# tavildar/Polar

Measured on AMD Instinct MI355X. Metric: codewords/s (N=2048 K=1024 L=32 LLR-SCL), higher is better.
Workload: dtype f64

## Files before the change

### include/polar_amd_debug.h

```cpp
#ifndef POLAR_AMD_DEBUG_H
#define POLAR_AMD_DEBUG_H
#include "polar_amd.h"
#ifdef __cplusplus
extern "C" {
#endif

int polar_debug_set(polar_code_t *h, const char *key, long value);
long polar_debug_get(const polar_code_t *h, const char *key);
int polar_debug_comm_inits(void);
int polar_debug_weak_leaves(const polar_code_t *h);
void *polar_debug_scratch_ptr(polar_code_t *h);

#ifdef __cplusplus
}
#endif
#endif
```

### polar_amd/csrc/polar_debug.cpp

```cpp
#include "polar_multi.h"
#include "polar_amd_debug.h"

extern "C" {

int polar_debug_weak_leaves(const polar_code_t *h) { return polar_get_weak_leaves(h); }

int polar_debug_set(polar_code_t *h, const char *key, long value) {
    if (!h || !key) return fail(POLAR_E_ARG, "NULL argument");
    polar_code::Knobs &k = h->knobs;
    const std::string s(key);
    if (s == "mode_override") { if (value < -1 || value > 2) return fail(POLAR_E_ARG, "mode_override must be -1 (none), 0, 1 or 2"); k.mode_override = (int)value; }
    else if (s == "sc_no_fold") k.sc_no_fold = value != 0;
    else if (s == "no_tables") k.no_tables = value != 0;
    else if (s == "no_fuse_front") k.no_fuse_front = value != 0;
    else if (s == "no_prefix") h->prefix_on = (value == 0);
    else if (s == "no_rccl") { k.no_rccl = value != 0; multi_release(h, false); }
    else if (s == "force_rccl") { k.force_rccl = value != 0; multi_release(h, false); }
#ifdef POLAR_TEST_HOOKS
    else if (s == "host_fail_alloc") k.host_fail_alloc = value;
    else if (s == "share_device") { k.share_device = value != 0; multi_release(h, false); }
    else if (s == "fail_device") k.fail_device = (int)value;
    else if (s == "fail_collective") k.fail_collective = (int)value;
#endif
    else if (s == "lat_max_b") k.lat_max_b = value;
    else if (s == "host_pipe_min_bytes") k.host_pipe_min_bytes = value;
    else if (s == "host_chunk_bytes") k.host_chunk_bytes = value;
    else if (s == "host_lanes") { if (value < 0 || value > HostPipe::kMaxLanes) return fail(POLAR_E_ARG, "host_lanes must be 0 (default) or 1 .. %d", HostPipe::kMaxLanes); k.host_lanes = value; }
    else if (s == "host_ramp") k.host_ramp = value;
    else if (s == "host_prefault") { if (value < -1 || value > 16) return fail(POLAR_E_ARG, "host_prefault must be -1 (none), 0 (default) or 1 .. 16 threads"); k.host_prefault = value; }
    else if (s == "host_threads") { if (value < 0) return fail(POLAR_E_ARG, "host_threads must be >= 0"); k.host_threads = value; }
    else if (s == "multi_grace_s") { if (value < 0) return fail(POLAR_E_ARG, "multi_grace_s must be >= 0"); k.multi_grace_s = value; }
#ifdef POLAR_TEST_HOOKS
    else if (s == "force_workers") { k.force_workers = value != 0; multi_release(h, false); }
    else if (s == "stall_device") k.stall_device = (int)value;
    else if (s == "stall_ms") { if (value < 0) return fail(POLAR_E_ARG, "stall_ms must be >= 0"); k.stall_ms = value; }
#endif
    else if (s == "multi_timeout_s") { if (value < 0) return fail(POLAR_E_ARG, "multi_timeout_s must be >= 0 (0 = no watchdog)"); k.multi_timeout_s = value; }
    else return fail(POLAR_E_ARG, "polar_debug_set: unknown key '%s'", key);
    drop_clones(h);
    return POLAR_OK;
}
void *polar_debug_scratch_ptr(polar_code_t *h) { return h ? (void *)h->d_llr_scr.p : nullptr; }
long polar_debug_get(const polar_code_t *h, const char *key) {
    if (!key) return -1;
    const std::string s(key);
    if (s == "allocs") return (long)g_allocs.load();
    if (s == "comm_inits") return (long)polar_debug_comm_inits();
// ... 4 lines not shown
#else
        return 0;
#endif
    }
    if (s == "weak_leaves") return h->weak_leaves;
    if (s == "mode_override") return h->knobs.mode_override;
    if (s == "last_rounds") return h->last_rounds;
    if (s == "last_round_max_per_device") return h->last_round_max_per_device;
    if (s == "worker_threads_started") return h->worker_threads_started;
    if (s.compare(0, 9, "round_us_") == 0) {
        if (h->round_us.empty()) return 0;
        std::vector<long> v(h->round_us);
        if (s == "round_us_count") return (long)v.size();
        if (s == "round_us_first") return v.front();
        std::sort(v.begin(), v.end());
        if (s == "round_us_min") return v.front();
        if (s == "round_us_max") return v.back();
        if (s == "round_us_median") return v[v.size() / 2];
        return -1;
    }
    if (s == "multi_poisoned") return h->multi_poisoned ? 1 : 0;
    if (s == "host_chunks") return h->hpipe ? h->hpipe->last_chunks : 0;
    if (s == "host_chunk_cw") return h->hpipe ? h->hpipe->last_chunk_cw : 0;
    if (s == "host_lanes") return h->hpipe ? h->hpipe->last_lanes : 0;
    if (s == "host_threads") return h->hpipe ? h->hpipe->last_threads : 0;
    if (s == "host_us_copy_in") return h->hpipe ? h->hpipe->us_copy_in : 0;
    if (s == "host_us_wait") return h->hpipe ? h->hpipe->us_wait : 0;
    if (s == "host_us_copy_out") return h->hpipe ? h->hpipe->us_copy_out : 0;
    if (s == "host_us_total") return h->hpipe ? h->hpipe->us_total : 0;
    return -1;
}
int polar_debug_comm_inits(void) { return g_comm_inits.load(); }

}
```

### polar_amd/csrc/polar_decode.cpp

```cpp
#include "polar_host.h"

namespace {

size_t scratch_budget(const polar_code *h) {
    size_t budget = (size_t)24 << 30, free_b = 0, total_b = 0;
    if (hipMemGetInfo(&free_b, &total_b) == hipSuccess) budget = std::min(budget, (free_b + h->d_llr_scr.cap * sizeof(double)) / 2);
    return std::max(budget, (size_t)64 << 20);
}
template <typename Ensure>
int grid_that_fits(const polar_code *h, long want, size_t per_wave, Ensure ensure, int *grid_out) {
    long grid = want;
    if ((size_t)want * per_wave > h->d_llr_scr.cap * sizeof(double)) grid = std::max<long>(1, std::min<long>(want, (long)(scratch_budget(h) / per_wave)));
    for (;;) {
        const int rc = ensure((int)grid);
        if (rc != POLAR_E_NOMEM || grid <= 64) { *grid_out = (int)grid; return rc; }
        (void)hipGetLastError();
        grid /= 2;
    }
}

}

extern "C" {

int polar_decode_scl_llr_batch_dev(polar_code_t *h, const double *d_llr, long B, int L, uint8_t *d_out,
                                   double *d_pm, void *stream) {
    return polar_decode_scl_llr_batch_dev_ev(h, d_llr, B, L, d_out, d_pm, stream, nullptr, nullptr);
}

}

bool polar_host::use_sc_lat(const polar_code *h, long B) {
    return h->n <= polar_sc_lat_max_log() && polar_sc_lat_lds_bytes(h->N, (int)h->sc_lat_ops.size()) <= h->lds_per_block &&
           h->knobs.lat_max_b >= 0 && B <= (h->knobs.lat_max_b ? h->knobs.lat_max_b : 2048);
}

extern "C" {

int polar_decode_scl_llr_batch_dev_ev(polar_code_t *h, const double *d_llr, long B, int L, uint8_t *d_out,
                                      double *d_pm, void *stream, void *ev_start, void *ev_stop) {
    return decode_impl(h, d_llr, 0, B, nullptr, L, d_out, d_pm, stream, ev_start, ev_stop);
}

}

int polar_host::decode_impl(polar_code *h, const void *d_llr, int llr_f32, long B, const unsigned int *n_dev, int L, uint8_t *d_out,
                            double *d_pm, void *stream, void *ev_start, void *ev_stop, int phase, int *deferred) {
    if (!h || !d_llr || !d_out) return fail(POLAR_E_ARG, "NULL argument");
    if (deferred) *deferred = 0;
    if (L < 1 || L > POLAR_MAX_LIST) return fail(POLAR_E_ARG, "list size %d out of range [1, %d]", L, POLAR_MAX_LIST);
    if (B < 0) return fail(POLAR_E_ARG, "negative batch");
    if (B == 0) return POLAR_OK;
    DevGuard dg_;
    int rc = ensure_device(h, dg_);
    if (rc) return rc;
    const int gs = pow2ceil(L);
    const int G = 64 / gs;
    int wpc = h->waves_per_cu ? h->waves_per_cu : 16;
    int lds_log_auto = 0;
    if (!h->waves_per_cu && !h->lds_log && gs >= 16 && (B + G - 1) / G <= (long)h->num_cu * 4 &&
        polar_decode_lds_bytes(5, 1) <= h->lds_per_block) { wpc = 4; lds_log_auto = 5; }
    const int pipe = (wpc > 8) ? 0 : 1;
    int lds_log = h->lds_log ? h->lds_log : (lds_log_auto ? lds_log_auto : (pipe ? 4 : 3));
    const int wpb = polar_decode_waves_per_block(pipe);
    const size_t lds = polar_decode_lds_bytes(lds_log, pipe);
    const int max_blocks_by_lds = (int)(h->lds_per_block / lds);
    if (max_blocks_by_lds < 1) return fail(POLAR_E_ARG, "lds_log %d does not fit the LDS", lds_log);
    if (wpc > max_blocks_by_lds * wpb) wpc = max_blocks_by_lds * wpb;
    long groups = (B + G - 1) / G;
    long maxgrid = (long)h->num_cu * wpc;
    int grid = (int)std::min(groups, maxgrid);
    grid = ((grid + wpb - 1) / wpb) * wpb;
    const int SL = 1 << lds_log;
    const size_t big = (h->N > 2 * SL) ? (size_t)(h->N - 2 * SL) : 0;
    const size_t cwords = (h->N >= 128) ? (size_t)(h->N / 32 - 2) : 0;
    if ((size_t)grid * big * 64 + 64 > h->d_llr_scr.cap) {
        const size_t per_wave = big * 64 * sizeof(double) + 1;
        const long cap = (long)(scratch_budget(h) / per_wave);
        if (grid > cap) grid = (int)std::max<long>(wpb, (cap / wpb) * wpb);
    }
    if ((rc = h->d_llr_scr.ensure((size_t)grid * big * 64 + 64))) return rc;
    if ((rc = h->d_c_scr.ensure((size_t)grid * 2 * cwords * 64 + 64))) return rc;
    if ((rc = h->d_hist_scr.ensure((size_t)grid * 3 * h->W * 64 + 64))) return rc;
    PolarDecodeParams p;
    p.n = h->n; p.N = h->N; p.K = h->K; p.crc = h->crc; p.L = L; p.W = h->W; p.B = B;
    {
        int P = 0;
        while (P < h->N && h->frozen[P]) ++P;
        int Q = 0;
        if (gs >= 4 && h->prefix_on) {
            if (P >= 256) Q = 256;
            else { Q = 64; while (Q <= P) Q <<= 1; if (P < 33) Q = 0; }
            if (Q > h->N / 2) Q = 0;
        }
        p.prefix_q = Q;
        p.prefix_len = Q ? std::min(P, Q) : 0;
    }
    p.llr = (const double *)d_llr; p.llr_f32 = llr_f32; p.p0 = nullptr; p.out = d_out; p.pm_out = d_pm;
    p.frozen = h->d_frozen.p; p.info_rank = h->d_info_rank.p; p.crc_mask = h->d_crc_mask.p; p.tabs = h->d_tabs.p;
    p.ctl = h->d_ctl.p;
    p.pre = nullptr;
    p.flags = nullptr; p.cw_list = nullptr; p.cw_count = nullptr; p.n_dev = n_dev;
    p.tab_scr = nullptr; p.var_scr = nullptr;
    if (p.prefix_q) {
        if ((rc = h->d_pre.ensure((size_t)B * (size_t)(h->N - p.prefix_q + 1)))) return rc;
        p.pre = h->d_pre.p;
    }
    p.llr_scr = h->d_llr_scr.p; p.c_scr = h->d_c_scr.p; p.hist_scr = h->d_hist_scr.p;
    if ((rc = h->d_work.ensure(1))) return rc;
    p.work = h->d_work.p;
    hipStream_t st = (hipStream_t)stream;
    const int mode = h->knobs.mode_override >= 0 ? h->knobs.mode_override : h->mode;
    if (L == 1 && mode != 1 && !d_pm) {
        const long groups8 = (B + 7) / 8;
        const int sgrid = (int)std::min<long>(groups8, (long)h->num_cu * polar_sc8_waves_per_cu(h->N));
        const bool fold = h->sc_fold && !h->knobs.sc_no_fold && ((uintptr_t)d_llr & 15u) == 0;
// ... 52 lines not shown
            if (ev_start) HIP_TRY(hipEventRecord((hipEvent_t)ev_start, st));
            HIP_TRY(polar_launch_decode_lat(pl, gs, lat_ed, blocks, st));
            if (ev_stop) HIP_TRY(hipEventRecord((hipEvent_t)ev_stop, st));
            if (!lat_ed) return POLAR_OK;
            if (phase == 1 && deferred) { *deferred = 2; return POLAR_OK; }
        } else if (!lat_ed) return POLAR_OK;
        HIP_TRY(hipMemsetAsync(h->d_count.p, 0, sizeof(unsigned int), st));
        HIP_TRY(polar_launch_ed_collect(h->d_flags.p, B, n_dev, h->d_list.p, h->d_count.p, st));
        HIP_TRY(hipMemsetAsync(p.work, 0, sizeof(unsigned int), st));
        PolarDecodeParams pf = p;
        pf.prefix_q = 0; pf.prefix_len = 0; pf.pre = nullptr;
        pf.cw_list = h->d_list.p; pf.cw_count = h->d_count.p; pf.n_dev = nullptr;
        HIP_TRY(polar_launch_decode_llr(pf, gs, lds_log, pipe, std::min(grid, 64 * wpb), false, st));
        return POLAR_OK;
    }
    HIP_TRY(hipMemsetAsync(p.work, 0, sizeof(unsigned int), st));
    if (!ed) {
        if (p.prefix_q) HIP_TRY(polar_launch_prefix(p, false, nullptr, st));
        if (ev_start) HIP_TRY(hipEventRecord((hipEvent_t)ev_start, st));
        HIP_TRY(polar_launch_decode_llr(p, gs, lds_log, pipe, grid, false, st));
        if (ev_stop) HIP_TRY(hipEventRecord((hipEvent_t)ev_stop, st));
        return POLAR_OK;
    }
    if ((rc = h->d_ech.ensure((size_t)B * h->N))) return rc;
    if ((rc = h->d_flags.ensure((size_t)B))) return rc;
    if ((rc = h->d_list.ensure((size_t)B))) return rc;
    if ((rc = h->d_count.ensure(1))) return rc;
    HIP_TRY(hipMemsetAsync(h->d_count.p, 0, sizeof(unsigned int), st));
    const bool fuse_front = p.prefix_q > 0 && polar_prefix_is_staged(h->N) && !h->knobs.no_fuse_front;
    if (!fuse_front) HIP_TRY(polar_launch_ed_front(d_llr, llr_f32, h->d_ech.p, h->d_flags.p, h->d_tabs.p, h->N, B, n_dev, st));
    PolarDecodeParams pe = p;
    pe.llr = h->d_ech.p; pe.llr_f32 = 0; pe.flags = h->d_flags.p;
    if (gs == 32 && !pipe && h->N >= 1024 && p.prefix_q > 0 && !h->knobs.no_tables) {
        if ((rc = h->d_tab_scr.ensure((size_t)grid * G * 3 * h->N + 64))) return rc;
        if ((rc = h->d_var_scr.ensure((size_t)grid * (h->N / 32) * 64 + 64))) return rc;
        pe.tab_scr = h->d_tab_scr.p; pe.var_scr = h->d_var_scr.p;
    }
    if (pe.prefix_q && fuse_front) {
        PolarDecodeParams pp = pe;
        pp.llr = (const double *)d_llr; pp.llr_f32 = llr_f32;
        HIP_TRY(polar_launch_prefix(pp, true, h->d_ech.p, st));
    } else if (pe.prefix_q) HIP_TRY(polar_launch_prefix(pe, true, nullptr, st));
    if (ev_start) HIP_TRY(hipEventRecord((hipEvent_t)ev_start, st));
    HIP_TRY(polar_launch_decode_llr(pe, gs, lds_log, pipe, grid, true, st));
    if (ev_stop) HIP_TRY(hipEventRecord((hipEvent_t)ev_stop, st));
    HIP_TRY(polar_launch_ed_collect(h->d_flags.p, B, n_dev, h->d_list.p, h->d_count.p, st));
    HIP_TRY(hipMemsetAsync(p.work, 0, sizeof(unsigned int), st));
    PolarDecodeParams pf = p;
    pf.prefix_q = 0; pf.prefix_len = 0; pf.pre = nullptr;
    pf.cw_list = h->d_list.p; pf.cw_count = h->d_count.p; pf.n_dev = nullptr;
    const int fgrid = h->weak_leaves ? grid : std::min(grid, 64 * wpb);
    HIP_TRY(polar_launch_decode_llr(pf, gs, lds_log, pipe, fgrid, false, st));
    return POLAR_OK;
}

extern "C" {

int polar_decode_scl_llr_batch_dev_f32(polar_code_t *h, const float *d_llr, long B, int L, uint8_t *d_out,
                                       double *d_pm, void *stream) {
    return decode_impl(h, d_llr, 1, B, nullptr, L, d_out, d_pm, stream, nullptr, nullptr);
}

int polar_decode_scl_p1_batch(polar_code_t *h, const double *p1, const double *p0, long B, int L, uint8_t *out) {
    if (!h || !p1 || !p0 || !out) return fail(POLAR_E_ARG, "NULL argument");
    if (L < 1 || L > POLAR_MAX_LIST) return fail(POLAR_E_ARG, "list size %d out of range [1, %d]", L, POLAR_MAX_LIST);
    if (B < 0) return fail(POLAR_E_ARG, "negative batch");
    if (B == 0) return POLAR_OK;
    DevGuard dg_;
    int rc = ensure_device(h, dg_);
    if (rc) return rc;
    const int N = h->N;
// ... 265 lines not shown
```

### polar_amd/csrc/polar_handle.cpp

```cpp
#include "polar_host.h"

namespace polar_host {

thread_local std::string g_err;

int fail(int code, const char *fmt, ...) {
    char buf[512];
    va_list ap;
    va_start(ap, fmt);
    vsnprintf(buf, sizeof buf, fmt, ap);
    va_end(ap);
    g_err = buf;
    return code;
}

std::atomic<unsigned long> g_allocs{0};

int usable_cpus() {
    int n = (int)std::thread::hardware_concurrency();
    cpu_set_t set;
    if (sched_getaffinity(0, sizeof set, &set) == 0) n = CPU_COUNT(&set);
    if (FILE *f = fopen("/sys/fs/cgroup/cpu.max", "r")) {
        char q[32]; long per = 0;
        if (fscanf(f, "%31s %ld", q, &per) == 2 && strcmp(q, "max") != 0 && per > 0) n = std::min<long>(n, std::max<long>(1, atol(q) / per));
// ... 161 lines not shown
        int v = 0;
        h->lds_per_block = (hipDeviceGetAttribute(&v, hipDeviceAttributeMaxSharedMemoryPerBlock, h->device) == hipSuccess && v > 0) ? (size_t)v : (size_t)64 * 1024;
    }
    int rc;
    if ((rc = upload(h->d_frozen, h->frozen))) return rc;
    if ((rc = upload(h->d_ctl, h->ctl))) return rc;
    if ((rc = upload(h->d_sc_ops, h->sc_ops))) return rc;
    if ((rc = upload(h->d_sc_lat_ops, h->sc_lat_ops))) return rc;
    if ((rc = upload(h->d_order, h->order))) return rc;
    if ((rc = upload(h->d_info_rank, h->info_rank))) return rc;
    if ((rc = upload(h->d_crc_mask, h->crc_mask))) return rc;
    if ((rc = upload(h->d_crcm, h->crcm))) return rc;
    {
        std::vector<double> t(322);
        for (int j = 0; j < 64; ++j) t[j] = j ? 2.0 * std::exp2(-(double)(64 - j) / 64.0) : 1.0;
        for (int j = 0; j <= 128; ++j) {
            t[64 + j] = 1.0 / (1.0 + (double)j / 128.0);
            t[64 + 129 + j] = std::log1p((double)j / 128.0);
        }
        if ((rc = upload(h->d_tabs, t))) return rc;
    }
    h->dev_ready = true;
    return POLAR_OK;
}

int read_env_knobs(polar_code *h) {
    auto on = [](const char *name) { const char *e = getenv(name); return e && *e && strcmp(e, "0") != 0; };
    if (const char *e = getenv("POLAR_MODE")) {
        if (!(e[0] >= '0' && e[0] <= '2' && e[1] == 0)) return fail(POLAR_E_ARG, "POLAR_MODE=%s: must be 0, 1 or 2", e);
        h->knobs.mode_override = e[0] - '0';
    }
    h->knobs.sc_no_fold = on("POLAR_SC_NO_FOLD");
    h->knobs.no_tables = on("POLAR_NO_TABLES");
    h->knobs.no_rccl = on("POLAR_NO_RCCL");
    h->knobs.force_rccl = on("POLAR_FORCE_RCCL");
    return POLAR_OK;
}

void drop_clones(polar_code *h) {
    if (h->multi_poisoned) return;
    for (polar_code *c : h->clones) polar_destroy(c);
    h->clones.clear();
    if (h->hpipe) for (polar_code *&c : h->hpipe->ctx) if (c) { polar_destroy(c); c = nullptr; }
}

}

extern "C" {

const char *polar_last_error(void) { return g_err.c_str(); }
int polar_version(void) { return 100; }

int polar_create(int n, int K, double eps, int crc, polar_code_t **out) {
    if (!out) return fail(POLAR_E_ARG, "out is NULL");
    if (n < 1 || n > POLAR_MAX_N_LOG2) return fail(POLAR_E_ARG, "n = %d out of range [1, %d]", n, POLAR_MAX_N_LOG2);
    const int N = 1 << n;
    if (K < 1 || crc < 0 || crc > POLAR_MAX_CRC || K + crc > N)
        return fail(POLAR_E_ARG, "need 1 <= K, 0 <= crc <= %d, K + crc <= N (K=%d crc=%d N=%d)", POLAR_MAX_CRC, K, crc, N);
    polar_code *h = new polar_code;
    h->n = n; h->N = N; h->K = K; h->crc = crc; h->eps = eps;
    make_bitrev(h);
    std::vector<double> z(N, eps);
    for (int it = 0; it < n; ++it) {
        const int inc = 1 << it;
        for (int j = 0; j < inc; ++j)
            for (int i = 0; i < N; i += 2 * inc) {
// ... 139 lines not shown
```

### polar_amd/csrc/polar_host.h

```cpp
#pragma once
#include <hip/hip_runtime.h>

#include <dlfcn.h>
#include <sched.h>
#include <sys/mman.h>
#include <unistd.h>

#include <algorithm>
#include <atomic>
#include <chrono>
#include <condition_variable>
#include <memory>
#include <mutex>
#include <thread>
#include <cmath>
#include <cstdarg>
#include <cstdio>
#include <cstdlib>
#include <cstring>
#include <functional>
#include <numeric>
#include <string>
#include <vector>

// ... 175 lines not shown
    std::vector<uint32_t> crc_mask;
    std::vector<uint8_t> sched;
    std::vector<uint32_t> ctl;
    int weak_leaves = 0;
    std::vector<uint32_t> sc_ops;
    std::vector<uint32_t> sc_lat_ops;
    bool sc_fold = false;
    bool dev_ready = false;
    int device = -1, num_cu = 0;
    size_t lds_per_block = 0;
    DevBuf<uint8_t> d_frozen, d_crcm;
    DevBuf<uint16_t> d_order, d_info_rank;
    DevBuf<uint32_t> d_crc_mask, d_ctl, d_sc_ops, d_sc_lat_ops, d_var_scr;
    DevBuf<double> d_tab_scr;
    DevBuf<unsigned int> d_flag_words;
    DevBuf<double> d_llr_scr, d_tabs, d_pre;
    DevBuf<uint32_t> d_c_scr, d_hist_scr;
    DevBuf<double> d_in;
    DevBuf<float> d_f32;
    DevBuf<uint8_t> d_out, d_bytes_a, d_bytes_b;
    DevBuf<unsigned long long> d_counter;
    DevBuf<unsigned int> d_work;
    DevBuf<uint64_t> d_sel;
    DevBuf<double> d_ech;
    DevBuf<uint8_t> d_flags;
    DevBuf<uint32_t> d_list;
    DevBuf<unsigned int> d_count;
    int mode = 0;
    struct Knobs {
        int mode_override = -1;
        bool sc_no_fold = false;
        bool no_tables = false;
        bool no_fuse_front = false;
        bool no_rccl = false;
        bool force_rccl = false;
        bool share_device = false;
        int fail_device = -1;
        int fail_collective = -1;
        long multi_timeout_s = 1800;
        long multi_grace_s = 10;
        bool force_workers = false;
        int stall_device = -1;
        long stall_ms = 0;
        long lat_max_b = 0;
        long host_pipe_min_bytes = 0;
        long host_chunk_bytes = 0;
        long host_lanes = 0;
        long host_threads = 0;
        long host_ramp = 0;
        long host_fail_alloc = 0;
        long host_prefault = 0;
    } knobs;
    DevBuf<uint64_t> d_alive[2];
    DevBuf<unsigned int> d_nalive;
    DevBuf<unsigned long long> d_mc_ctr;
    struct McSlot { DevBuf<uint64_t> list[2]; int cur = 0; long cnt = 0; };
    std::vector<McSlot> mc_slots;
    DevBuf<unsigned int> d_slot_n;
    std::vector<unsigned int> h_slot_n;
    std::vector<polar_code *> clones;
    struct MultiCtx *multi = nullptr;
    bool multi_poisoned = false;
    bool ctx_stuck = false;
    void *pin_in = nullptr, *pin_in_dev = nullptr;
    uint8_t *pin_out = nullptr, *pin_out_dev = nullptr;
    size_t pin_in_cap = 0, pin_out_cap = 0;
    uint8_t *lat_flag_bytes = nullptr;
    struct HostPipe *hpipe = nullptr;
    long last_rounds = 0, last_round_max_per_device = 0, worker_threads_started = 0;
    std::vector<long> round_us;
    int waves_per_cu = 0, lds_log = 0, pipe = -1;
    bool prefix_on = true;
};

namespace polar_host {

struct DevGuard {
    int prev = -1;
    ~DevGuard() { if (prev >= 0) (void)hipSetDevice(prev); }
};

inline int pow2ceil(int v) { int p = 1; while (p < v) p <<= 1; return p; }

int derive_tables(polar_code *h);
int ensure_device(polar_code *h, DevGuard &dg);
void drop_clones(polar_code *h);
template <typename T>
int upload(DevBuf<T> &d, const std::vector<T> &v) {
    size_t n = v.size() ? v.size() : 1;
    int rc = d.ensure(n);
    if (rc) return rc;
    if (v.size()) HIP_TRY(hipMemcpy(d.p, v.data(), v.size() * sizeof(T), hipMemcpyHostToDevice));
    return POLAR_OK;
}
int decode_impl(polar_code *h, const void *d_llr, int llr_f32, long B, const unsigned int *n_dev, int L, uint8_t *d_out,
                double *d_pm, void *stream, void *ev_start, void *ev_stop, int phase = 0, int *deferred = nullptr);
bool use_sc_lat(const polar_code *h, long B);
void fill_enc(const polar_code *h, PolarEncodeParams &p);
int mlc_check(const polar_code *h, int constellation, int *cid);
void fill_mlc(const polar_code *h, int cid, double snr_db, PolarMlcParams &p);
int mlc_decode_launch(polar_code *h, int cid, const double *d_y, double n0, long B, const unsigned int *n_dev, double *d_out,
                      uint8_t *d_out_bytes, hipStream_t st);
void hostpipe_release(polar_code *h);
void multi_release(polar_code *h, bool abort_comms);
polar_code *copy_ctx(polar_code *h, int dev);
polar_code *clone_on_device(polar_code *h, int dev, bool fresh = false);

}
```

### polar_amd/csrc/polar_kernels.h

```cpp
#pragma once
#include <hip/hip_runtime.h>
#include <stdint.h>
#include <stddef.h>

struct PolarDecodeParams {
    int n, N, K, crc, L;
    int W;
    int prefix_q, prefix_len;
    long B;
    const double *llr;
    int llr_f32;
    const double *p0;
    uint8_t *out;
    double *pm_out;
    const uint8_t *frozen;
    const uint32_t *ctl;
    unsigned int *work;
    const uint16_t *info_rank;
    const uint32_t *crc_mask;
    const double *tabs;
    const double *pre;
    double *llr_scr;
    uint32_t *c_scr;
    uint32_t *hist_scr;
    uint8_t *flags;
    const uint32_t *cw_list;
    const unsigned int *cw_count;
    const unsigned int *n_dev;
    double *tab_scr;
    uint32_t *var_scr;
};

size_t polar_decode_lds_bytes(int lds_log, int pipe);
int polar_decode_waves_per_block(int pipe);
hipError_t polar_launch_prefix(const PolarDecodeParams &p, bool ed, double *ech_out, hipStream_t st);
hipError_t polar_launch_prefix_ed0(const PolarDecodeParams &p, double *ech_out, hipStream_t st);
hipError_t polar_launch_prefix_ed1(const PolarDecodeParams &p, double *ech_out, hipStream_t st);
int polar_prefix_is_staged(int N);
hipError_t polar_launch_decode_llr_ed0(const PolarDecodeParams &p, int gs, int lds_log, int pipe, int grid, hipStream_t st);
hipError_t polar_launch_decode_llr_ed1(const PolarDecodeParams &p, int gs, int lds_log, int pipe, int grid, hipStream_t st);
hipError_t polar_launch_decode_lat(const PolarDecodeParams &p, int gs, bool ed, int blocks, hipStream_t st);
size_t polar_decode_lat_lds_bytes(int N, int gs, int W);
hipError_t polar_launch_decode_llr(const PolarDecodeParams &p, int gs, int lds_log, int pipe, int grid, bool ed, hipStream_t st);
hipError_t polar_launch_ed_front(const void *llr, int llr_f32, double *ech, uint8_t *flags, const double *tabs, int N, long B, const unsigned *n_dev, hipStream_t st);
hipError_t polar_launch_ed_collect(const uint8_t *flags, long B, const unsigned *n_dev, uint32_t *list, unsigned *count, hipStream_t st);

hipError_t polar_launch_decode_p1(const PolarDecodeParams &p, int gs, int grid, hipStream_t st);

struct PolarScP1Params {
    int n, N, K;
    long B;
    const double *p1;
    double *out;
    const uint8_t *frozen;
    const uint16_t *order;
    double *scr;
};
hipError_t polar_launch_sc_p1(const PolarScP1Params &p, int grid, hipStream_t st);
hipError_t polar_launch_sc_p1_lat(const PolarScP1Params &p, int grid, hipStream_t st);
size_t polar_sc_p1_lat_lds_bytes(int N);

struct PolarScParams {
    int n, N, K;
    long B;
    const double *ech_t;
    const void *llr;
    int llr_f32;
    uint8_t *out;
    const uint32_t *ops;
    int n_ops;
    const uint16_t *order;
// ... 130 lines not shown
```

### polar_amd/csrc/polar_kernels.hip

```cpp
#include <hip/hip_runtime.h>
#include <stdint.h>
#include <type_traits>

#include "polar_kernels.h"
#include "polar_device.h"
#include "polar_edom.h"

#ifdef POLAR_PROFILE
#define PROF_DECL u64 prof_acc[24] = {0,0,0,0,0,0,0,0,0,0,0,0,0,0,0,0,0,0,0,0,0,0,0,0}; u64 prof_t = __builtin_readcyclecounter();
#define PROF(i) { u64 t_ = __builtin_readcyclecounter(); prof_acc[i] += t_ - prof_t; prof_t = t_; }
#define PROF_OUT if (lane == 0 && p.pm_out) { for (int i_ = 0; i_ < 24; ++i_) atomicAdd((u64 *)p.pm_out + i_, prof_acc[i_]); }
#define PROF_CNT(i, v) { prof_acc[i] += (u64)(v); }
#else
#define PROF_DECL
#define PROF(i)
#define PROF_CNT(i, v)
#define PROF_OUT
#endif

#include "polar_llr_nodes.h"

template <bool ED>
__device__ __forceinline__ const double *ch_row(const PolarDecodeParams &p, size_t cw, int N) {
    return p.llr_f32 ? reinterpret_cast<const double *>(reinterpret_cast<const float *>(p.llr) + cw * (size_t)N)
                     : p.llr + cw * (size_t)N;
}
#define CH(row, i) (p.llr_f32 ? (double)reinterpret_cast<const float *>(row)[i] : (row)[i])

#ifndef FU
#define FU 4
#endif
#ifndef POLAR_SKIP_L1
#define POLAR_SKIP_L1 1
#endif
#define POLAR_SADDR 1
#ifndef OCC
#define OCC 4
#endif
#define LANE_CTX                                   \
    const int lane = LAT ? lane_k : lane_id_opaque();    \
    const int lig = lane & (GS - 1);               \
    const int gbase = lane & ~(GS - 1);            \
    (void)lig; (void)gbase;
template <int GS, int LDS_LOG, int PIPE, bool ED, int NL = 0, int LAT = 0>
__global__ __launch_bounds__(PIPE ? 64 : 256, PIPE ? 2 : OCC) void scl_decode_llr_kernel(PolarDecodeParams p) {
    constexpr int WPB = PIPE ? 1 : 4;
    constexpr int G = LAT ? 1 : 64 / GS;
    constexpr int EL = 64 / GS;
    constexpr int CST = LAT ? GS : 64;
#define POLAR_CL (LAT ? lig : lane)
#define POLAR_CGB (LAT ? 0 : gbase)
    constexpr int SL = 1 << LDS_LOG;
    const int lane = threadIdx.x & 63;
    const int wib = __builtin_amdgcn_readfirstlane((int)(threadIdx.x >> 6));
    const int wave_id = blockIdx.x * WPB + wib;
    const int nwaves = gridDim.x * WPB;
    const int lane_k = lane;
    (void)lane_k;
    const int lig = lane & (GS - 1);
    const int gbase = lane & ~(GS - 1);
    const int grp = LAT ? 0 : lane / GS;
    const int n = NL ? NL : p.n, N = NL ? (1 << NL) : p.N, K = p.K, L = p.L;
    const u64 gmask = (GS == 64) ? ~0ull : ((1ull << GS) - 1ull);

    extern __shared__ __attribute__((aligned(16))) unsigned char smem[];
    double *tabs = reinterpret_cast<double *>(smem);
    constexpr size_t WAVE_LDS = (size_t)(2 * SL - 1) * 64 * 8 + 128 * 8 + 128;
    unsigned char *wbase = smem + 324 * 8 + (size_t)wib * WAVE_LDS;
    double *lds_llr = reinterpret_cast<double *>(wbase);
    double *sortbuf = lds_llr + (LAT ? 0 : (size_t)(2 * SL - 1) * 64);
    unsigned char *stackv = reinterpret_cast<unsigned char *>(sortbuf + 128);
    unsigned char *srcof = stackv + 64;
    for (int i = threadIdx.x; i < 322; i += WPB * 64) tabs[i] = p.tabs[i];
    if (WPB > 1) __syncthreads();
    const Tabs tb = {tabs, tabs + 64, tabs + 64 + 129};
    u64 guard = 0;
    double gacc = __builtin_inf();
    auto FN = [&](double a, double b) -> double {
        if constexpr (ED) return f_node_e_acc(a, b, gacc); else return f_node(a, b, tb);
    };
    auto GN = [&](double a, double b, uint32_t cw_, int bi) -> double {
        if constexpr (ED) return g_node_e(a, b, cw_ << (31 - bi), tb); else return g_node(a, b, (cw_ >> bi) & 1u);
    };
    const long Bv = p.cw_count ? (long)*p.cw_count : (p.n_dev ? ((long)*p.n_dev < p.B ? (long)*p.n_dev : p.B) : p.B);

    const size_t big_elems = (N > 2 * SL) ? (size_t)(N - 2 * SL) : 0;
    double *g_llr = LAT ? nullptr : p.llr_scr + (size_t)wave_id * big_elems * 64;
    const int cwords = (N >= 128) ? (N / 32 - 2) : 0;
    double *lat_ch = reinterpret_cast<double *>(stackv + 128);
    double *lat_a = lat_ch + N;
    uint32_t *lat_w = reinterpret_cast<uint32_t *>(lat_a + (size_t)N * GS);
    uint32_t *g_cl = LAT ? lat_w : p.c_scr + (size_t)wave_id * 2 * (size_t)cwords * 64;
    uint32_t *g_cr = g_cl + (size_t)cwords * CST;
    uint32_t *g_hist = LAT ? g_cr + (size_t)cwords * CST : p.hist_scr + (size_t)wave_id * 3 * (size_t)p.W * 64;
    uint32_t *g_horg = g_hist + (size_t)p.W * CST;
    uint32_t *g_tb = g_horg + (size_t)p.W * CST;
    const int S1 = N / 2, S2 = N / 4;
    const bool tbl = ED && !PIPE && GS == 32 && N >= 1024 && p.tab_scr != nullptr && p.prefix_q > 0;
    double *tab_w = tbl ? p.tab_scr + (size_t)wave_id * G * (size_t)(3 * N) : nullptr;
    uint32_t *g_v = tbl ? p.var_scr + (size_t)wave_id * (size_t)(S2 / 8) * 64 : nullptr;

    for (long g0 = (long)wave_id * G; g0 < Bv;) {
        const long cwi = g0 + grp;
        const bool valid = (cwi < Bv);
        const long cw = (p.cw_list && valid) ? (long)p.cw_list[cwi] : cwi;
        guard = 0;
        gacc = __builtin_inf();
        auto cw_of_lane = [&](int ln) -> size_t {
            const long i = g0 + (LAT ? 0 : ln / GS);
            return p.cw_list ? (size_t)p.cw_list[i < Bv ? i : Bv - 1] : (size_t)i;
        };
        auto FN2 = [&](double a0_, double b0_, double a1_, double b1_, double &r0_, double &r1_) {
            if constexpr (ED) { r0_ = f_node_e_acc(a0_, b0_, gacc); r1_ = f_node_e_acc(a1_, b1_, gacc); }
            else f_node2(a0_, b0_, a1_, b1_, tb, r0_, r1_);
        };

        bool active = valid && (lig == L - 1);
        u64 actw = __ballot(active);
        double pm = 0.0;
        int sp = L - 1;
        if (lig < L - 1) stackv[gbase + lig] = (unsigned char)lig;
        P16 pL = {0, 0};
        P16 pC = {0, 0};
        u64 clsmall = 0;
        uint32_t hword = 0;
        int origin = lig;
        unsigned t = 0;
        if constexpr (LAT) {
            bool any = false, sized = false;
            const size_t row = (size_t)(valid ? cw : 0) * (size_t)N;
            for (int i0 = 0; i0 < N; i0 += 64 * 8) {
                double x[8];
#pragma unroll
                for (int k = 0; k < 8; ++k) {
                    const int i = i0 + 64 * k + lane;
                    x[k] = (i < N) ? (p.llr_f32 ? (double)reinterpret_cast<const float *>(p.llr)[row + i] : p.llr[row + i]) : 1.0;
                }
#pragma unroll
                for (int k = 0; k < 8; ++k) {
                    const int i = i0 + 64 * k + lane;
// ... 382 lines not shown
    long blocks = (B + 3) / 4;
    if (blocks > 16384) blocks = 16384;
    if (llr_f32) hipLaunchKernelGGL(ed_front_kernel<float>, dim3((unsigned)blocks), dim3(256), 0, st, (const float *)llr, ech, flags, tabs, N, B, n_dev);
    else hipLaunchKernelGGL(ed_front_kernel<double>, dim3((unsigned)blocks), dim3(256), 0, st, (const double *)llr, ech, flags, tabs, N, B, n_dev);
    return hipGetLastError();
}
__global__ __launch_bounds__(256) void ed_collect_kernel(const uint8_t *flags, long B, const unsigned *n_dev, uint32_t *list, unsigned *count) {
    if (n_dev && (long)*n_dev < B) B = (long)*n_dev;
    for (long cw = (long)blockIdx.x * 256 + threadIdx.x; cw < B; cw += (long)gridDim.x * 256)
        if (flags[cw]) list[atomicAdd(count, 1u)] = (uint32_t)cw;
}
hipError_t polar_launch_ed_collect(const uint8_t *flags, long B, const unsigned *n_dev, uint32_t *list, unsigned *count, hipStream_t st) {
    long blocks = (B + 255) / 256;
    if (blocks > 1024) blocks = 1024;
    hipLaunchKernelGGL(ed_collect_kernel, dim3((unsigned)blocks), dim3(256), 0, st, flags, B, n_dev, list, count);
    return hipGetLastError();
}

int polar_decode_waves_per_block(int pipe) { return pipe ? 1 : 4; }
size_t polar_decode_lds_bytes(int lds_log, int pipe) {
    return 324 * 8 + (size_t)polar_decode_waves_per_block(pipe) * ((size_t)((2u << lds_log) - 1) * 64 * 8 + 128 * 8 + 128);
}

#endif

template <int GS, bool ED>
static hipError_t launch_gs(const PolarDecodeParams &p, int lds_log, int pipe, int grid, hipStream_t st) {
    size_t lds = polar_decode_lds_bytes(lds_log, pipe);
    const int wpb = polar_decode_waves_per_block(pipe);
#define POLAR_LAUNCH(LL, PP) hipLaunchKernelGGL((scl_decode_llr_kernel<GS, LL, PP, ED>), dim3(grid / wpb), dim3(64 * wpb), lds, st, p)
#ifndef POLAR_NO_FIXED_N
    if constexpr (GS == 32 && ED) {
        if (lds_log == 3 && !pipe && (p.n == 11 || p.n == 10)) {
            if (p.n == 11) hipLaunchKernelGGL((scl_decode_llr_kernel<GS, 3, 0, ED, 11>), dim3(grid / wpb), dim3(64 * wpb), lds, st, p);
            else hipLaunchKernelGGL((scl_decode_llr_kernel<GS, 3, 0, ED, 10>), dim3(grid / wpb), dim3(64 * wpb), lds, st, p);
            return hipGetLastError();
        }
    }
#endif
    switch (lds_log * 2 + (pipe ? 1 : 0)) {
        case 6: POLAR_LAUNCH(3, 0); break;
#ifndef POLAR_DEV_ONE
        case 4: POLAR_LAUNCH(2, 0); break;
        case 7: POLAR_LAUNCH(3, 1); break;
        case 8: POLAR_LAUNCH(4, 0); break;
        case 9: POLAR_LAUNCH(4, 1); break;
        case 10: POLAR_LAUNCH(5, 0); break;
        case 11: POLAR_LAUNCH(5, 1); break;
#endif
        default: return hipErrorInvalidValue;
    }
#undef POLAR_LAUNCH
    return hipGetLastError();
}

template <int GS, bool ED>
static hipError_t launch_lat(const PolarDecodeParams &p, int blocks, hipStream_t st) {
    const size_t lds = polar_decode_lat_lds_bytes(p.N, GS, p.W);
    const hipError_t e = hipFuncSetAttribute(reinterpret_cast<const void *>(&scl_decode_llr_kernel<GS, 3, 1, ED, 0, 1>), hipFuncAttributeMaxDynamicSharedMemorySize, (int)lds);
    if (e != hipSuccess) return e;
    hipLaunchKernelGGL((scl_decode_llr_kernel<GS, 3, 1, ED, 0, 1>), dim3(blocks), dim3(64), lds, st, p);
    return hipGetLastError();
}
#if POLAR_ED_TU == 3
hipError_t polar_launch_decode_lat_ed1(const PolarDecodeParams &p, int gs, int blocks, hipStream_t st) {
    switch (gs) {
        case 2: return launch_lat<2, true>(p, blocks, st);
        case 4: return launch_lat<4, true>(p, blocks, st);
        case 8: return launch_lat<8, true>(p, blocks, st);
        default: return hipErrorInvalidValue;
    }
}
#elif POLAR_ED_TU == 0
hipError_t polar_launch_decode_lat_ed1(const PolarDecodeParams &p, int gs, int blocks, hipStream_t st);
hipError_t polar_launch_decode_lat(const PolarDecodeParams &p, int gs, bool ed, int blocks, hipStream_t st) {
    if (ed) return polar_launch_decode_lat_ed1(p, gs, blocks, st);
    if (gs == 2) return launch_lat<2, false>(p, blocks, st);
    return hipErrorInvalidValue;
}
size_t polar_decode_lat_lds_bytes(int N, int gs, int W) {
    const int cwords = (N >= 128) ? (N / 32 - 2) : 0;
    return 324 * 8 + (128 * 8 + 128) + (size_t)N * 8 + (size_t)N * gs * 8 + ((size_t)2 * cwords + (size_t)3 * W) * gs * 4 + 64;
}
#endif

#if POLAR_ED_TU == 2
hipError_t polar_launch_decode_llr_ed1_gs32(const PolarDecodeParams &p, int lds_log, int pipe, int grid, hipStream_t st) {
    return launch_gs<32, true>(p, lds_log, pipe, grid, st);
}
#elif POLAR_ED_TU == 1
hipError_t polar_launch_decode_llr_ed1_gs32(const PolarDecodeParams &p, int lds_log, int pipe, int grid, hipStream_t st);
hipError_t polar_launch_decode_llr_ed1(const PolarDecodeParams &p, int gs, int lds_log, int pipe, int grid, hipStream_t st) {
    switch (gs) {
#ifndef POLAR_DEV_GS32
        case 4: return launch_gs<4, true>(p, lds_log, pipe, grid, st);
        case 8: return launch_gs<8, true>(p, lds_log, pipe, grid, st);
        case 16: return launch_gs<16, true>(p, lds_log, pipe, grid, st);
        case 64: return launch_gs<64, true>(p, lds_log, pipe, grid, st);
#endif
        case 32: return polar_launch_decode_llr_ed1_gs32(p, lds_log, pipe, grid, st);
        default: return hipErrorInvalidValue;
    }
}
#elif POLAR_ED_TU == 0
hipError_t polar_launch_decode_llr_ed0(const PolarDecodeParams &p, int gs, int lds_log, int pipe, int grid, hipStream_t st) {
    switch (gs) {
        case 1: return launch_gs<1, false>(p, lds_log, pipe, grid, st);
#ifndef POLAR_DEV_GS32
        case 2: return launch_gs<2, false>(p, lds_log, pipe, grid, st);
        case 4: return launch_gs<4, false>(p, lds_log, pipe, grid, st);
        case 8: return launch_gs<8, false>(p, lds_log, pipe, grid, st);
        case 16: return launch_gs<16, false>(p, lds_log, pipe, grid, st);
        case 64: return launch_gs<64, false>(p, lds_log, pipe, grid, st);
#endif
        case 32: return launch_gs<32, false>(p, lds_log, pipe, grid, st);
        default: return hipErrorInvalidValue;
    }
}
hipError_t polar_launch_decode_llr(const PolarDecodeParams &p, int gs, int lds_log, int pipe, int grid, bool ed, hipStream_t st) {
// ... 4 lines not shown
```

Before: 1.034 million.

## Fuse prefix computation into decode kernel and pick balanced persistent grid

```diff
diff --git a/include/polar_amd_debug.h b/include/polar_amd_debug.h
--- a/include/polar_amd_debug.h
+++ b/include/polar_amd_debug.h
@@ -10,6 +10,8 @@
 int polar_debug_comm_inits(void);
 int polar_debug_weak_leaves(const polar_code_t *h);
 void *polar_debug_scratch_ptr(polar_code_t *h);
+int polar_debug_read_pre(polar_code_t *h, long cw0, long rows, long row_len, double *out);
+long polar_debug_persistent_grid(long groups, long resident, int waves_per_block);
 
 #ifdef __cplusplus
 }
diff --git a/polar_amd/csrc/polar_debug.cpp b/polar_amd/csrc/polar_debug.cpp
--- a/polar_amd/csrc/polar_debug.cpp
+++ b/polar_amd/csrc/polar_debug.cpp
@@ -13,6 +13,7 @@
     else if (s == "sc_no_fold") k.sc_no_fold = value != 0;
     else if (s == "no_tables") k.no_tables = value != 0;
     else if (s == "no_fuse_front") k.no_fuse_front = value != 0;
+    else if (s == "no_inkernel_prefix") k.no_inkernel_prefix = value != 0;
     else if (s == "no_prefix") h->prefix_on = (value == 0);
     else if (s == "no_rccl") { k.no_rccl = value != 0; multi_release(h, false); }
     else if (s == "force_rccl") { k.force_rccl = value != 0; multi_release(h, false); }
@@ -83,4 +84,29 @@
 }
 int polar_debug_comm_inits(void) { return g_comm_inits.load(); }
 
+int polar_debug_read_pre(polar_code_t *h, long cw0, long rows, long row_len, double *out) {
+#ifdef POLAR_TEST_HOOKS
+    if (!h || !out || cw0 < 0 || rows < 0 || row_len <= 0) return fail(POLAR_E_ARG, "polar_debug_read_pre: bad argument");
+    if ((size_t)(cw0 + rows) * (size_t)row_len > h->d_pre.cap) return fail(POLAR_E_ARG, "polar_debug_read_pre: rows beyond the prefix buffer of the last decode");
+    DevGuard dg_;
+    int rc = ensure_device(h, dg_);
+    if (rc) return rc;
+    HIP_TRY(hipDeviceSynchronize());
+    HIP_TRY(hipMemcpy(out, h->d_pre.p + (size_t)cw0 * (size_t)row_len, (size_t)rows * (size_t)row_len * sizeof(double), hipMemcpyDeviceToHost));
+    return POLAR_OK;
+#else
+    (void)h; (void)cw0; (void)rows; (void)row_len; (void)out;
+    return fail(POLAR_E_ARG, "polar_debug_read_pre exists in the test build only");
+#endif
 }
+long polar_debug_persistent_grid(long groups, long resident, int waves_per_block) {
+#ifdef POLAR_TEST_HOOKS
+    if (waves_per_block < 1) return -1;
+    return persistent_grid(groups, resident, waves_per_block);
+#else
+    (void)groups; (void)resident; (void)waves_per_block;
+    return -1;
+#endif
+}
+
+}
diff --git a/polar_amd/csrc/polar_decode.cpp b/polar_amd/csrc/polar_decode.cpp
--- a/polar_amd/csrc/polar_decode.cpp
+++ b/polar_amd/csrc/polar_decode.cpp
@@ -19,6 +19,17 @@
     }
 }
 
+}
+
+long polar_host::persistent_grid(long groups, long resident, int wpb) {
+    if (groups <= 0 || resident <= 0) return 0;
+    if (groups <= resident) return groups;
+    const long top = (resident / wpb) * wpb;
+    for (long g = top; g >= wpb; g -= wpb) {
+        const long r = groups % g;
+        if (r == 0 || 4 * r >= 3 * g) return g;
+    }
+    return top > 0 ? top : resident;
 }
 
 extern "C" {
@@ -71,6 +82,7 @@
     long maxgrid = (long)h->num_cu * wpc;
     int grid = (int)std::min(groups, maxgrid);
     grid = ((grid + wpb - 1) / wpb) * wpb;
+    const int grid_full = grid;
     const int SL = 1 << lds_log;
     const size_t big = (h->N > 2 * SL) ? (size_t)(h->N - 2 * SL) : 0;
     const size_t cwords = (h->N >= 128) ? (size_t)(h->N / 32 - 2) : 0;
@@ -82,6 +94,9 @@
     if ((rc = h->d_llr_scr.ensure((size_t)grid * big * 64 + 64))) return rc;
     if ((rc = h->d_c_scr.ensure((size_t)grid * 2 * cwords * 64 + 64))) return rc;
     if ((rc = h->d_hist_scr.ensure((size_t)grid * 3 * h->W * 64 + 64))) return rc;
+    const int grid_scr = grid;
+    if (grid == grid_full && groups > grid)
+        grid = (int)((persistent_grid(groups, grid, wpb) + wpb - 1) / wpb) * wpb;
     PolarDecodeParams p;
     p.n = h->n; p.N = h->N; p.K = h->K; p.crc = h->crc; p.L = L; p.W = h->W; p.B = B;
     {
@@ -200,11 +215,13 @@
     PolarDecodeParams pe = p;
     pe.llr = h->d_ech.p; pe.llr_f32 = 0; pe.flags = h->d_flags.p;
     if (gs == 32 && !pipe && h->N >= 1024 && p.prefix_q > 0 && !h->knobs.no_tables) {
-        if ((rc = h->d_tab_scr.ensure((size_t)grid * G * 3 * h->N + 64))) return rc;
-        if ((rc = h->d_var_scr.ensure((size_t)grid * (h->N / 32) * 64 + 64))) return rc;
+        if ((rc = h->d_tab_scr.ensure((size_t)grid_scr * G * 3 * h->N + 64))) return rc;
+        if ((rc = h->d_var_scr.ensure((size_t)grid_scr * (h->N / 32) * 64 + 64))) return rc;
         pe.tab_scr = h->d_tab_scr.p; pe.var_scr = h->d_var_scr.p;
     }
-    if (pe.prefix_q && fuse_front) {
+    const bool ink = fuse_front && pe.tab_scr && !h->knobs.no_inkernel_prefix && polar_decode_has_inkernel_prefix(gs, lds_log, pipe, h->n);
+    if (ink) { pe.raw = d_llr; pe.raw_f32 = llr_f32; }
+    else if (pe.prefix_q && fuse_front) {
         PolarDecodeParams pp = pe;
         pp.llr = (const double *)d_llr; pp.llr_f32 = llr_f32;
         HIP_TRY(polar_launch_prefix(pp, true, h->d_ech.p, st));
diff --git a/polar_amd/csrc/polar_handle.cpp b/polar_amd/csrc/polar_handle.cpp
--- a/polar_amd/csrc/polar_handle.cpp
+++ b/polar_amd/csrc/polar_handle.cpp
@@ -217,6 +217,7 @@
     }
     h->knobs.sc_no_fold = on("POLAR_SC_NO_FOLD");
     h->knobs.no_tables = on("POLAR_NO_TABLES");
+    h->knobs.no_inkernel_prefix = on("POLAR_NO_INKERNEL_PREFIX");
     h->knobs.no_rccl = on("POLAR_NO_RCCL");
     h->knobs.force_rccl = on("POLAR_FORCE_RCCL");
     return POLAR_OK;
diff --git a/polar_amd/csrc/polar_host.h b/polar_amd/csrc/polar_host.h
--- a/polar_amd/csrc/polar_host.h
+++ b/polar_amd/csrc/polar_host.h
@@ -231,6 +231,7 @@
         bool sc_no_fold = false;
         bool no_tables = false;
         bool no_fuse_front = false;
+        bool no_inkernel_prefix = false;
         bool no_rccl = false;
         bool force_rccl = false;
         bool share_device = false;
@@ -295,6 +296,7 @@
 int decode_impl(polar_code *h, const void *d_llr, int llr_f32, long B, const unsigned int *n_dev, int L, uint8_t *d_out,
                 double *d_pm, void *stream, void *ev_start, void *ev_stop, int phase = 0, int *deferred = nullptr);
 bool use_sc_lat(const polar_code *h, long B);
+long persistent_grid(long groups, long resident, int wpb);
 void fill_enc(const polar_code *h, PolarEncodeParams &p);
 int mlc_check(const polar_code *h, int constellation, int *cid);
 void fill_mlc(const polar_code *h, int cid, double snr_db, PolarMlcParams &p);
diff --git a/polar_amd/csrc/polar_kernels.h b/polar_amd/csrc/polar_kernels.h
--- a/polar_amd/csrc/polar_kernels.h
+++ b/polar_amd/csrc/polar_kernels.h
@@ -29,6 +29,8 @@
     const unsigned int *n_dev;
     double *tab_scr;
     uint32_t *var_scr;
+    const void *raw = nullptr;
+    int raw_f32 = 0;
 };
 
 size_t polar_decode_lds_bytes(int lds_log, int pipe);
@@ -37,6 +39,7 @@
 hipError_t polar_launch_prefix_ed0(const PolarDecodeParams &p, double *ech_out, hipStream_t st);
 hipError_t polar_launch_prefix_ed1(const PolarDecodeParams &p, double *ech_out, hipStream_t st);
 int polar_prefix_is_staged(int N);
+int polar_decode_has_inkernel_prefix(int gs, int lds_log, int pipe, int n);
 hipError_t polar_launch_decode_llr_ed0(const PolarDecodeParams &p, int gs, int lds_log, int pipe, int grid, hipStream_t st);
 hipError_t polar_launch_decode_llr_ed1(const PolarDecodeParams &p, int gs, int lds_log, int pipe, int grid, hipStream_t st);
 hipError_t polar_launch_decode_lat(const PolarDecodeParams &p, int gs, bool ed, int blocks, hipStream_t st);
diff --git a/polar_amd/csrc/polar_kernels.hip b/polar_amd/csrc/polar_kernels.hip
--- a/polar_amd/csrc/polar_kernels.hip
+++ b/polar_amd/csrc/polar_kernels.hip
@@ -27,6 +27,98 @@
 }
 #define CH(row, i) (p.llr_f32 ? (double)reinterpret_cast<const float *>(row)[i] : (row)[i])
 
+template <int NLOG, int TABS_BYTES, int WAVE_BYTES>
+__device__ __attribute__((noinline)) void inkernel_prefix(const PolarDecodeParams &p, long g0, long Bv, int wib) {
+    extern __shared__ __attribute__((aligned(16))) unsigned char smem[];
+    constexpr int n = NLOG, N = 1 << NLOG, S0 = N / 2;
+    static_assert(WAVE_BYTES >= S0 * 8 + 128, "the staging row is the wave's layer area + exchange buffer");
+    const double *tabs = reinterpret_cast<const double *>(smem);
+    const Tabs tb = {tabs, tabs + 64, tabs + 64 + 129};
+    double *stg = reinterpret_cast<double *>(smem + TABS_BYTES + (size_t)wib * WAVE_BYTES);
+    const int Q = p.prefix_q, Pe = p.prefix_len;
+    const int ln = lane_id_opaque();
+#pragma unroll 1
+    for (int k = 0; k < 2; ++k) {
+        if (g0 + k >= Bv) break;
+        const size_t cwk = (size_t)(g0 + k);
+        double *prow = const_cast<double *>(p.pre) + cwk * (size_t)(N - Q + 1);
+        double *erow = const_cast<double *>(p.llr) + cwk * (size_t)N;
+        const size_t rbase = cwk * (size_t)N;
+        auto RAW = [&](int i) -> double {
+            return p.raw_f32 ? (double)reinterpret_cast<const float *>(p.raw)[rbase + (size_t)i]
+                             : reinterpret_cast<const double *>(p.raw)[rbase + (size_t)i];
+        };
+        u64 pguard = 0;
+        bool any = false, sized = false;
+#pragma unroll 1
+        for (int m = ln; m < S0; m += 512) {
+            double x0[8], x1[8];
+#pragma unroll
+            for (int q = 0; q < 8; ++q) { x0[q] = RAW(2 * (m + 64 * q)); x1[q] = RAW(2 * (m + 64 * q) + 1); }
+#pragma unroll
+            for (int q = 0; q < 8; ++q) {
+                const int mq = m + 64 * q;
+                bool f0, f1;
+                const double a = ed_from_channel(x0[q], tb, f0), b = ed_from_channel(x1[q], tb, f1);
+                any |= f0 | f1;
+                sized |= (fabs(x0[q]) >= 0.1) | (fabs(x1[q]) >= 0.1);
+                erow[2 * mq] = a; erow[2 * mq + 1] = b;
+                stg[__brev((unsigned)mq) >> (33 - n)] = f_node_e(a, b, pguard);
+            }
+        }
+        wave_mem_fence();
+#pragma unroll 8
+        for (int j = ln; j < S0; j += 64) prow[1 + j] = stg[j];
+#pragma unroll 1
+        for (int S = S0 / 2; S >= Q; S >>= 1) {
+            double *outp = prow + 1 + (size_t)(N - 2 * S);
+#pragma unroll 2
+            for (int j = ln; j < S; j += 64) {
+                const double r = f_node_e(stg[j], stg[j + S], pguard);
+                stg[j] = r;
+                outp[j] = r;
+            }
+            wave_mem_fence();
+        }
+#pragma unroll 1
+        for (int h = Q / 2; h >= 1; h >>= 1) {
+#pragma unroll 1
+            for (int pi = ln; pi < Q / 2; pi += 64) {
+                const int i = ((pi & ~(h - 1)) << 1) | (pi & (h - 1));
+                const double lo = stg[i], hi = stg[i + h];
+                stg[i] = f_node_e(lo, hi, pguard);
+                stg[i + h] = g_node_e(lo, hi, 0u, tb);
+            }
+            wave_mem_fence();
+        }
+#pragma unroll 1
+        for (int i = ln; i < Pe; i += 64) {
+            bool ng; double al, sneg, spos;
+            leaf_terms<true>(stg[i], true, __builtin_amdgcn_ballot_w64(true), tb, ng, al, sneg, spos);
+            stg[i] = ng ? spos : sneg;
+        }
+        wave_mem_fence();
+        double acc = 0.0;
+        int c = 0;
+#pragma unroll 1
+        for (; c + 16 <= Pe; c += 16) {
+            double t[16];
+#pragma unroll
+            for (int q = 0; q < 16; ++q) t[q] = stg[c + q];
+#pragma unroll
+            for (int q = 0; q < 16; ++q) acc = acc + t[q];
+        }
+#pragma unroll 1
+        for (; c < Pe; ++c) acc = acc + stg[c];
+        const bool bad_in = wave_any(any) || !wave_any(sized);
+        if (ln == 0) {
+            prow[0] = acc;
+            p.flags[cwk] = (pguard != 0 || bad_in) ? 1 : 0;
+        }
+        wave_mem_fence();
+    }
+}
+
 #ifndef FU
 #define FU 4
 #endif
@@ -42,11 +134,13 @@
     const int lig = lane & (GS - 1);               \
     const int gbase = lane & ~(GS - 1);            \
     (void)lig; (void)gbase;
-template <int GS, int LDS_LOG, int PIPE, bool ED, int NL = 0, int LAT = 0>
+template <int GS, int LDS_LOG, int PIPE, bool ED, int NL = 0, int LAT = 0, int INKP = 0>
 __global__ __launch_bounds__(PIPE ? 64 : 256, PIPE ? 2 : OCC) void scl_decode_llr_kernel(PolarDecodeParams p) {
     constexpr int WPB = PIPE ? 1 : 4;
     constexpr int G = LAT ? 1 : 64 / GS;
     constexpr int EL = 64 / GS;
+    constexpr bool INK = INKP != 0;
+    static_assert(!INK || (ED && GS == 32 && !PIPE && !LAT && NL == 11 && LDS_LOG == 3), "in-kernel prefix: exp-domain list of 32 at N = 2048 only");
     constexpr int CST = LAT ? GS : 64;
 #define POLAR_CL (LAT ? lig : lane)
 #define POLAR_CGB (LAT ? 0 : gbase)
@@ -106,6 +200,7 @@
         const long cw = (p.cw_list && valid) ? (long)p.cw_list[cwi] : cwi;
         guard = 0;
         gacc = __builtin_inf();
+        if constexpr (INK) inkernel_prefix<NL, (int)(324 * 8), (int)WAVE_LDS>(p, g0, Bv, wib);
         auto cw_of_lane = [&](int ln) -> size_t {
             const long i = g0 + (LAT ? 0 : ln / GS);
             return p.cw_list ? (size_t)p.cw_list[i < Bv ? i : Bv - 1] : (size_t)i;
@@ -554,7 +649,8 @@
 #ifndef POLAR_NO_FIXED_N
     if constexpr (GS == 32 && ED) {
         if (lds_log == 3 && !pipe && (p.n == 11 || p.n == 10)) {
-            if (p.n == 11) hipLaunchKernelGGL((scl_decode_llr_kernel<GS, 3, 0, ED, 11>), dim3(grid / wpb), dim3(64 * wpb), lds, st, p);
+            if (p.n == 11 && p.raw) hipLaunchKernelGGL((scl_decode_llr_kernel<GS, 3, 0, ED, 11, 0, 1>), dim3(grid / wpb), dim3(64 * wpb), lds, st, p);
+            else if (p.n == 11) hipLaunchKernelGGL((scl_decode_llr_kernel<GS, 3, 0, ED, 11>), dim3(grid / wpb), dim3(64 * wpb), lds, st, p);
             else hipLaunchKernelGGL((scl_decode_llr_kernel<GS, 3, 0, ED, 10>), dim3(grid / wpb), dim3(64 * wpb), lds, st, p);
             return hipGetLastError();
         }
@@ -607,6 +703,13 @@
 #endif
 
 #if POLAR_ED_TU == 2
+int polar_decode_has_inkernel_prefix(int gs, int lds_log, int pipe, int n) {
+#ifndef POLAR_NO_FIXED_N
+    return (gs == 32 && lds_log == 3 && !pipe && n == 11) ? 1 : 0;
+#else
+    return 0;
+#endif
+}
 hipError_t polar_launch_decode_llr_ed1_gs32(const PolarDecodeParams &p, int lds_log, int pipe, int grid, hipStream_t st) {
     return launch_gs<32, true>(p, lds_log, pipe, grid, st);
 }
```

After: 552,700. -46.6%, worse.
